# bxh1/VIDO-SLAM

Measured on AMD Instinct MI355X. Metric: frames/sec end-to-end (flow+depth+track+local-BA) at 640x480; BA iters/sec, higher is better.
Workload: dtype f32

## Files before the change

### include/vido_c.h

```cpp
#ifndef VIDO_C_H
#define VIDO_C_H
#include <stdint.h>
#include <stddef.h>
#ifdef __cplusplus
extern "C" {
#endif

#define VIDO_OK              0
#define VIDO_E_INVALID      -1
#define VIDO_E_NO_DEVICE    -2
#define VIDO_E_HIP          -3
#define VIDO_E_CAPACITY     -4
#define VIDO_E_NOMEM        -5

#define VIDO_MAX_LEVELS 16

typedef struct vido_ctx vido_ctx;

typedef struct vido_keypoint { float x, y, size, angle, response; int32_t octave; } vido_keypoint;

typedef struct vido_config {
    int32_t device;
    int32_t width, height;
    int32_t max_batch;
// ... 179 lines not shown
int vido_mask_logit_select_n(vido_ctx* ctx, const float* feat, const float* w, const float* b, const long long* labels, float* out, int n, int c, int hw, int classes, const int32_t* n_live);
int vido_bias_act(vido_ctx* ctx, float* x, const float* bias, int N, int C, int H, int W, float slope);
int vido_bias_unary(vido_ctx* ctx, float* x, const float* bias, int N, int C, int H, int W, int kind);
int vido_upcat_reflect(vido_ctx* ctx, const float* x, const float* skip, int C1, int C2, int h, int w, float* out);
int vido_minmax_norm_u16(vido_ctx* ctx, const float* d, const float* mm, int64_t n, int32_t* out);
int vido_bias_res_act(vido_ctx* ctx, float* x, const float* bias, const float* res, int N, int C, int H, int W, float slope);
int vido_area_feed(vido_ctx* ctx, const uint8_t* bgr, int H, int W, float* out, int OH, int OW, float div);
int vido_backwarp(vido_ctx* ctx, const float* x, const float* flow, int B, int C, int H, int W, float* out);
int vido_deconv4s2_depthwise(vido_ctx* ctx, const float* x, const float* weight, int B, int C, int H, int W, float input_slope, float* out);

int vido_conv1x1_supported(int cin, int cout, int hw);
int vido_conv1x1_layout(int cin, int cout, int hw);
int vido_conv1x1_set_arith(int arith);
int vido_conv1x1_range_flag(vido_ctx* ctx, int reset);
int vido_range_latch(vido_ctx* ctx, unsigned* dst);
int vido_conv1x1_bias_act(vido_ctx* ctx, const float* x, const float* w_packed, const float* bias, const float* residual, float* y, int cin, int cout, int hw, float slope);
int vido_deconv2x2_supported(int n, int cin, int cout, int h, int w);
int vido_deconv2x2_bias_act(vido_ctx* ctx, const float* x, const float* w_packed, const float* bias, float* y, int n, int cin, int cout, int h, int w, float slope);
int vido_deconv2x2_bias_act_n(vido_ctx* ctx, const float* x, const float* w_packed, const float* bias, float* y, int n, int cin, int cout, int h, int w, float slope, const int32_t* n_live);
int vido_conv1x1_bias_up2_act(vido_ctx* ctx, const float* x, const float* w_packed, const float* bias, const float* residual_half, float* y, int cin, int cout, int h, int w, float slope);

int vido_conv_kxk_c2(vido_ctx* ctx, const float* x, const float* w, const float* bias, const float* residual, float* y, int cin, int k, int h, int w_);
int vido_conv1x1_skinny(vido_ctx* ctx, const float* x, const float* w_packed, const float* bias, const float* residual, float* y, int cin, int cout, long long hw, float slope);
int vido_stem7x7s2_pool(vido_ctx* ctx, const float* x, const float* w_packed, const float* bias, float* y, int h, int w);

int vido_conv_direct_supported(int cin, int cout, int h, int w, int kh, int kw, int sh, int sw, int ph, int pw);
long long vido_conv_direct_packed_floats(int cin, int cout, int kh, int kw);
int vido_conv_direct_pack(const float* w, int cin, int cout, int kh, int kw, float* w_packed);
int vido_conv_direct_bias_act(vido_ctx* ctx, const float* x, const float* w_packed, const float* bias, float* y, int n, int cin, int cout, int h, int w,
                              int kh, int kw, int sh, int sw, int ph, int pw, float slope);

int vido_wino3x3_supported(int cin, int cout, int h, int w);
int vido_wino3x3_fills_chip(int n, int cout, int h, int w, int min_wgs);
long long vido_wino3x3_packed_floats(int cin, int cout);
int vido_wino3x3_pack(const float* w, int cin, int cout, float* u_packed);
int vido_wino3x3_bias_act(vido_ctx* ctx, const float* x, const float* u_packed, const float* bias, float* y, int n, int cin, int cout, int h, int w, float slope);
int vido_wino3x3_form(int n, int cin, int cout, int h, int w);
int vido_fc_h_splitk(int rows, int k, int outs);
int vido_fc_h(vido_ctx* ctx, const float* x, const void* w_packed, const float* bias, float* part, float* y, int rows, int k, int outs, float slope);
int vido_conv3x3_h_supported(int n, int cin, int cout, int h, int w);
int vido_conv3x3_h_workgroups(int n, int cout, int h, int w);
int vido_conv3x3_h_bias_act(vido_ctx* ctx, const float* x, const void* w_packed, const float* bias, float* y, int n, int cin, int cout, int h, int w, float slope);
int vido_conv3x3_h_bias_act_n(vido_ctx* ctx, const float* x, const void* w_packed, const float* bias, float* y, int n, int cin, int cout, int h, int w, float slope, const int32_t* n_live);
int vido_conv3x3_h_live_form(int n, int cout, int h, int w, int live, int* channels, int* block_rows);
int vido_mask_head_coarse(void);
int vido_conv3x3_h_bias_act_form(vido_ctx* ctx, const float* x, const void* w_packed, const float* bias, float* y, int n, int cin, int cout, int h, int w, float slope, int rpw, int cg);
long long vido_wino3x3_packed_floats_form(int cin, int cout, int form);
int vido_wino3x3_pack_form(const float* w, int cin, int cout, int form, float* u_packed);
int vido_wino3x3_bias_act_form(vido_ctx* ctx, const float* x, const float* u_packed, const float* bias, float* y, int n, int cin, int cout, int h, int w, float slope, int form);
int vido_gconv3x3_supported(int H, int W, int cpg_in, int cpg_out);
int64_t vido_gconv3x3_packed_size(int groups, int cpg_in, int cpg_out);
int vido_gconv3x3_bias_act(vido_ctx* ctx, const float* x, const float* in_bias, const float* w_packed, const float* bias, float* y, int groups, int cpg_in, int cpg_out, int H, int W, float slope);
int vido_gconv3x3_s2_supported(int H, int W, int cpg_in, int cpg_out);
int vido_gconv3x3_s2_bias_act(vido_ctx* ctx, const float* x, const float* w_packed, const float* bias, float* y, int groups, int cpg_in, int cpg_out, int H, int W, float slope);
int vido_lfn_reg_front(vido_ctx* ctx, const float* im1, const float* im2, const float* flow, const float* mean, float scale, int B, int C, int H, int W, float* out, int out_channels);
int vido_lfn_reg_tail(vido_ctx* ctx, const float* dist, const float* flow, const float* wx, const float* bx, const float* wy, const float* by, int B, int K, int H, int W, float* out);
int vido_roi_align(vido_ctx* ctx, const float* feat, int B, int C, int H, int W, const float* rois, int n_rois,
                   float spatial_scale, int pooled_h, int pooled_w, int sampling_ratio, float* out, int on_device);
int vido_nms(vido_ctx* ctx, const float* boxes_xyxy, const float* scores, int n, float thresh, int32_t* keep_out,
             int32_t* n_keep, int on_device);
int vido_nms_grouped(vido_ctx* ctx, const float* boxes_xyxy, const float* scores, const int32_t* groups, int n, float thresh,
                     int32_t* keep_out, int32_t* n_keep, int on_device);
int vido_nms_segments(vido_ctx* ctx, const float* boxes_xyxy, const int32_t* groups, const int32_t* seg_off, const int32_t* seg_n, int n_seg, int max_n, int total,
                      float thresh, int32_t* keep_out, int32_t* n_keep);
int vido_roi_align_fpn(vido_ctx* ctx, const float* const feat[4], const int H[4], const int W[4], const float scale[4], int C, const float* boxes, const int32_t* level,
                       int n, int pooled_h, int pooled_w, int sampling_ratio, float* out);
int vido_nchw_to_nhwc(vido_ctx* ctx, const float* src, int B, int C, int H, int W, float* dst);
int vido_roi_align_fpn_nhwc(vido_ctx* ctx, const float* const feat[4], const int H[4], const int W[4], const float scale[4], int C, const float* boxes, const int32_t* level,
                            int n, int pooled_h, int pooled_w, int sampling_ratio, float* out);
// ... 97 lines not shown
```

### vido-slam_amd/csrc/conv3x3h.hip

```cpp
#include "common.hpp"
#include <type_traits>

namespace {
typedef float f32x16 __attribute__((ext_vector_type(16)));
typedef float f32x2 __attribute__((ext_vector_type(2)));
typedef _Float16 f16x8 __attribute__((ext_vector_type(8)));
typedef _Float16 f16x2 __attribute__((ext_vector_type(2)));
typedef unsigned u32x4 __attribute__((ext_vector_type(4)));

#define C3_OOB 0x40000000u
#define C3_WSLOT 24576
#define C3_RBW 3
#define C3_WPIX(BR) (((BR) + 2) * 18)
#define C3_XP(BR) ((16 * C3_WPIX(BR) + 511) / 512)
#define C3_RAW(BR) (C3_XP(BR) * 8 * 256)
#define C3_PLANE(BR) (C3_WPIX(BR) * 32)
#define C3_PBUF(BR) (2 * C3_PLANE(BR))
#define C3_LDS(BR) (C3_RBW * C3_WSLOT + C3_RAW(BR) + 2 * C3_PBUF(BR))

struct C3Args { const float* x; const void* wp; const float* bias; float* y; int N, Cin, Cout, H, W, nby, nbx, mt, total, nchunk; float slope; unsigned wbytes; unsigned* range_flag; const int* n_live; };

template <int RPW, int CG>
__device__ __forceinline__ void c3_body(const C3Args& A, const int nby, const int nbx, const int mt, const int total, const int per)
{
    constexpr int BR = 16 / CG, MT = 32 * RPW * CG, WPIX = C3_WPIX(BR), XP = C3_XP(BR), RAWB = C3_RAW(BR), PLANE = C3_PLANE(BR), PBUF = C3_PBUF(BR), CK = (WPIX * 8 + 511) / 512, NMM = 9 * RPW, NRD = 2 * RPW + 2;
    extern __shared__ __attribute__((aligned(16))) char c3_lds[];
    char* L = c3_lds;
    const int tid = threadIdx.x, lane = tid & 63, w = __builtin_amdgcn_readfirstlane(tid >> 6);
    const int q8 = blockIdx.x >> 3, item = (blockIdx.x & 7) * per + q8;
    if (q8 >= per || item >= total) return;
    const int nt = item / mt, mtile = item - nt * mt, m0 = mtile * MT;
    const int bpi = nby * nbx, n = nt / bpi, brem = nt - n * bpi, by = brem / nbx, bx = brem - by * nbx, Y0 = by * BR, X0 = bx * 16;
    const int rp = CG == 1 ? w : (w & 3), rb0 = CG == 1 ? 0 : RPW * (w >> 2);
    const int hw = A.H * A.W, nsteps = A.nchunk * 3;

    const __amdgpu_buffer_rsrc_t wr = __builtin_amdgcn_make_buffer_rsrc((void*)A.wp, 0, A.wbytes, 0x00020000);
    const unsigned avo = 16u * (unsigned)lane;
    unsigned abase[3], avq[3];
#pragma unroll
    for (int q = 0; q < 3; q++) { const int i = w + 8 * q, rb = i / 6, rem = i - 6 * rb; abase[q] = 1024u * (unsigned)(((m0 >> 5) + rb) * A.nchunk * 18 + rem); avq[q] = rb < RPW * CG ? avo : 0x80000000u; }
    unsigned xvo[11];
#pragma unroll
    for (int j = 0; j < XP; j++) {
        const int e = 64 * (8 * j + w) + lane, ch = e / WPIX, rem = e - ch * WPIX, row = rem / 18, col = rem - row * 18, gy = Y0 - 1 + row, gx = X0 - 1 + col;
        xvo[j] = (e < 16 * WPIX && gy >= 0 && gy < A.H && gx >= 0 && gx < A.W) ? 4u * (unsigned)(ch * hw + gy * A.W + gx) : C3_OOB;
    }
    const unsigned ximg = 4u * (unsigned)n * (unsigned)A.Cin * (unsigned)hw, ximg_end = ximg + 4u * (unsigned)A.Cin * (unsigned)hw, xchunk = 64u * (unsigned)hw;
    char* const RAW = L + C3_RBW * C3_WSLOT;
    char* const PL = RAW + RAWB;
    auto issue_w = [&](int s, int slot) {
        char* S = L + slot * C3_WSLOT + w * 1024;
        const unsigned so = 6144u * (unsigned)s;
// ... 103 lines not shown
    const bool inside = Y < A.H && X < A.W;
    float* yb = A.y + (size_t)n * A.Cout * hw + (size_t)Y * A.W + X;
#pragma unroll
    for (int rb = 0; rb < RPW; rb++) {
        float bv[16], sv[16];
#pragma unroll
        for (int r = 0; r < 16; r++) { const int co = m0 + 32 * (rb0 + rb) + 8 * (r >> 2) + 4 * (lane >> 5) + (r & 3); bv[r] = A.bias ? A.bias[co] : 0.f; sv[r] = wsc[co]; }
        if (inside) {
#pragma unroll
            for (int r = 0; r < 16; r++) {
                const int co = m0 + 32 * (rb0 + rb) + 8 * (r >> 2) + 4 * (lane >> 5) + (r & 3);
                const float v = acc[rb][r] * sv[r] + bv[r];
                yb[(size_t)co * hw] = fmaxf(v, v * A.slope);
            }
        }
    }
}

template <int RPW, int CG>
__global__ __launch_bounds__(512) void k_conv3x3_h(C3Args A)
{
    int total = A.total, per = gridDim.x >> 3;
    if (A.n_live) { const int nl = min(max(*A.n_live, 0), A.N); total = nl * A.nby * A.nbx * A.mt; per = (total + 7) >> 3; }
    c3_body<RPW, CG>(A, A.nby, A.nbx, A.mt, total, per);
}

#define C3_FINE_RPW 1
#define C3_FINE_CG 2
template <int RPWC, int CGC>
__global__ __launch_bounds__(512) void k_conv3x3_h_live(C3Args A, int fine_max)
{
    constexpr int BRF = 16 / C3_FINE_CG, MTF = 32 * C3_FINE_RPW * C3_FINE_CG, BRC = 16 / CGC, MTC = 32 * RPWC * CGC;
    const int nl = min(max(*A.n_live, 0), A.N), nbx = (A.W + 15) >> 4;
    const int nbyf = (A.H + BRF - 1) / BRF, mtf = A.Cout / MTF, tf = nl * nbyf * nbx * mtf;
    if (tf <= fine_max) c3_body<C3_FINE_RPW, C3_FINE_CG>(A, nbyf, nbx, mtf, tf, (tf + 7) >> 3);
    else { const int nbyc = (A.H + BRC - 1) / BRC, mtc = A.Cout / MTC, tc = nl * nbyc * nbx * mtc; c3_body<RPWC, CGC>(A, nbyc, nbx, mtc, tc, (tc + 7) >> 3); }
}
}

extern "C" {

int vido_conv3x3_h_supported(int n, int cin, int cout, int h, int w)
{
    const long long cp = (cin + 15) / 16 * 16;
    return n >= 1 && cin >= 1 && (cout == 32 || cout == 64 || (cout >= 128 && cout % 128 == 0)) && h >= 1 && w >= 1 && 4ll * n * cin * h * w < (1ll << 30) && 4ll * n * cout * h * w < (1ll << 30)
           && 36ll * cp * cout < (1ll << 31);
}

#define C3_MIN16 190
static int c3_block_rows(int n, int cout, int h, int w)
{
    static const int force = [] { const char* e = getenv("VIDO_CONV3X3_H_ROWS"); return e ? atoi(e) : 0; }();
    if (cout == 32) return 16;
    if (force == 16 || force == 8) return force;
    const int mt = cout >= 128 ? cout / 128 : 1;
    return n * ((h + 15) / 16) * ((w + 15) / 16) * mt >= C3_MIN16 ? 16 : 8;
}
int vido_conv3x3_h_workgroups(int n, int cout, int h, int w) { const int br = c3_block_rows(n, cout, h, w); return n * ((h + br - 1) / br) * ((w + 15) / 16) * (cout >= 128 ? cout / 128 : 1); }

// ... 67 lines not shown
    return VIDO_OK;
}

int vido_conv3x3_h_bias_act_form(vido_ctx* ctx, const float* x, const void* w_packed, const float* bias, float* y, int n, int cin, int cout, int h, int w, float slope, int rpw, int cg)
{
    if (!ctx) return VIDO_E_INVALID;
    const int MT = 32 * rpw * cg, form = rpw * 10 + cg;
    if (!x || !w_packed || !y || x == y || !vido_conv3x3_h_supported(n, cin, cout, h, w) || slope < 0.f || slope > 1.f || (((uintptr_t)x | (uintptr_t)y) & 3) || ((uintptr_t)w_packed & 15)
        || (form != 41 && form != 22 && form != 21 && form != 12 && form != 11) || cout % MT)
        return vido_set_error(ctx, VIDO_E_INVALID, "conv3x3_h_form: no kernel <%d, %d> for %d x %d -> %d channels at %d x %d", rpw, cg, n, cin, cout, h, w);
    HIP_TRY(ctx, hipSetDevice(ctx->device));
    { int rc = c3_set_attrs(ctx); if (rc) return rc; }
    hipStream_t st = ctx->has_ext_stream ? ctx->ext_stream : ctx->stream;
    const int br = 16 / cg, nby = (h + br - 1) / br, nbx = (w + 15) / 16, mt = cout / MT, total = n * nby * nbx * mt, nchunk = (cin + 15) / 16;
    C3Args A{x, w_packed, bias, y, n, cin, cout, h, w, nby, nbx, mt, total, nchunk, slope, (unsigned)(36ll * 16 * nchunk * cout), ctx->c1_range_flag, nullptr};
    const dim3 grid(8 * ((total + 7) / 8));
#define C3_LAUNCH(RPW_, CG_) hipLaunchKernelGGL((k_conv3x3_h<RPW_, CG_>), grid, dim3(512), C3_LDS(16 / CG_), st, A)
    if (form == 41) C3_LAUNCH(4, 1); else if (form == 22) C3_LAUNCH(2, 2); else if (form == 21) C3_LAUNCH(2, 1); else if (form == 12) C3_LAUNCH(1, 2); else C3_LAUNCH(1, 1);
#undef C3_LAUNCH
    HIP_TRY(ctx, hipGetLastError());
    return VIDO_OK;
}

}
```

### vido-slam_amd/csrc/convsmall.hip

```cpp
#include "common.hpp"

namespace {
template <int K>
__global__ __launch_bounds__(256) void k_conv_kxk_c2(const float* __restrict__ x, const float* __restrict__ w, const float* __restrict__ bias, const float* __restrict__ res,
                                                     float* __restrict__ y, int Cin, int H, int W)
{
    constexpr int R = K / 2, TS = 16 + K - 1, CC = 8, NT = CC * TS * TS, NL = (NT + 255) / 256, NW = (CC * K * K * 2 + 255) / 256;
    __shared__ float tile[NT];
    __shared__ __attribute__((aligned(8))) float wl[NW * 256];
    const int tid = threadIdx.x, tx = tid & 15, ty = tid >> 4, bx = blockIdx.x * 16, by = blockIdx.y * 16;
    const size_t HW = (size_t)H * W;
    int toff[NL]; bool tin[NL]; int tch[NL];
#pragma unroll
    for (int j = 0; j < NL; j++) {
        const int i = min(tid + 256 * j, NT - 1), c = i / (TS * TS), r = i - c * (TS * TS), yy = r / TS, xx = r - yy * TS, gy = by + yy - R, gx = bx + xx - R;
        tch[j] = c; tin[j] = tid + 256 * j < NT && gy >= 0 && gy < H && gx >= 0 && gx < W;
        toff[j] = min(max(gy, 0), H - 1) * W + min(max(gx, 0), W - 1);
    }
    float tv[NL], wv[NW];
    auto fetch = [&](int c0) {
#pragma unroll
        for (int j = 0; j < NL; j++) { const int c = min(c0 + tch[j], Cin - 1); tv[j] = x[(size_t)c * HW + toff[j]]; }
#pragma unroll
        for (int j = 0; j < NW; j++) {
// ... 14 lines not shown
#pragma unroll 2
        for (int c = 0; c < CC; c++) {
            const float* tc = tile + c * TS * TS + ty * TS + tx;
            const float2* wc = (const float2*)wl + c * K * K;
#pragma unroll
            for (int dy = 0; dy < K; dy++)
#pragma unroll
                for (int dx = 0; dx < K; dx++) {
                    const float v = tc[dy * TS + dx];
                    const float2 ww = wc[dy * K + dx];
                    acc0 = fmaf(v, ww.x, acc0); acc1 = fmaf(v, ww.y, acc1);
                }
        }
    }
    const int gy = by + ty, gx = bx + tx;
    if (gy < H && gx < W) {
        const size_t o = (size_t)gy * W + gx;
        y[o] = acc0 + (res ? res[o] : 0.f); y[HW + o] = acc1 + (res ? res[HW + o] : 0.f);
    }
}

typedef float f32x16s __attribute__((ext_vector_type(16)));
template <int CB, bool RES, int D>
__global__ __launch_bounds__(256) void k_conv1x1_skinny(const float* __restrict__ x, const float* __restrict__ wp, const float* __restrict__ bias, const float* __restrict__ res,
                                                        float* __restrict__ y, int Cin, int Cout, long long HW, float slope, unsigned xbytes, unsigned wbytes)
{
    const int lane = threadIdx.x & 63, wv = __builtin_amdgcn_readfirstlane(threadIdx.x >> 6);
    const long long p0 = ((long long)blockIdx.x * 4 + wv) * 32;
    if (p0 >= HW) return;
    const long long p = min(p0 + (lane & 31), HW - 1);
    const int nkp = Cin >> 1;
    f32x16s acc[CB];
#pragma unroll
    for (int cb = 0; cb < CB; cb++)
#pragma unroll
        for (int r = 0; r < 16; r++) acc[cb][r] = 0.f;
    const __amdgpu_buffer_rsrc_t xr = __builtin_amdgcn_make_buffer_rsrc((void*)x, 0, xbytes, 0x00020000);
    const __amdgpu_buffer_rsrc_t wr = __builtin_amdgcn_make_buffer_rsrc((void*)wp, 0, wbytes, 0x00020000);
    const unsigned xvo = 4u * (unsigned)((lane >> 5) * HW + p), wvo = 4u * (unsigned)lane;
    const unsigned hw8 = 8u * (unsigned)HW;
    float b[D], a[D][CB], bn[D], an[D][CB];
    auto fetch = [&](int kp0, float (&fb)[D], float (&fa)[D][CB]) {
#pragma unroll
        for (int u = 0; u < D; u++) {
            const int kp = min(kp0 + u, nkp - 1);
            fb[u] = __builtin_bit_cast(float, __builtin_amdgcn_raw_buffer_load_b32(xr, xvo, hw8 * (unsigned)kp, 0));
#pragma unroll
            for (int cb = 0; cb < CB; cb++) fa[u][cb] = __builtin_bit_cast(float, __builtin_amdgcn_raw_buffer_load_b32(wr, wvo, 256u * (unsigned)(cb * nkp + kp), 0));
        }
    };
    constexpr bool AHEAD = D > 4;
// ... 13 lines not shown
                b[u] = bn[u];
#pragma unroll
                for (int cb = 0; cb < CB; cb++) a[u][cb] = an[u][cb];
            }
        }
    }
    if (p0 + (lane & 31) < HW) {
#pragma unroll
        for (int cb = 0; cb < CB; cb++) {
            float bv[16], rv[16];
#pragma unroll
            for (int r = 0; r < 16; r++) {
                const int co = min(cb * 32 + 8 * (r >> 2) + 4 * (lane >> 5) + (r & 3), Cout - 1);
                bv[r] = bias ? bias[co] : 0.f; rv[r] = RES ? res[(size_t)co * HW + p] : 0.f;
            }
#pragma unroll
            for (int r = 0; r < 16; r++) {
                const int co = cb * 32 + 8 * (r >> 2) + 4 * (lane >> 5) + (r & 3);
                const float v = acc[cb][r] + bv[r] + rv[r];
                if (co < Cout) y[(size_t)co * HW + p] = fmaxf(v, v * slope);
            }
        }
    }
}
}

extern "C" {

int vido_conv_kxk_c2(vido_ctx* ctx, const float* x, const float* w, const float* bias, const float* residual, float* y, int cin, int k, int h, int wd)
{
    if (!ctx) return VIDO_E_INVALID;
    if (!x || !w || !y || x == y || cin < 1 || h < 1 || wd < 1 || (k != 3 && k != 5 && k != 7)) return vido_set_error(ctx, VIDO_E_INVALID, "conv_kxk_c2: bad arguments (k = %d)", k);
    HIP_TRY(ctx, hipSetDevice(ctx->device));
    hipStream_t st = ctx->has_ext_stream ? ctx->ext_stream : ctx->stream;
    const dim3 grid((wd + 15) / 16, (h + 15) / 16), blk(256);
    if (k == 7) hipLaunchKernelGGL(k_conv_kxk_c2<7>, grid, blk, 0, st, x, w, bias, residual, y, cin, h, wd);
    else if (k == 5) hipLaunchKernelGGL(k_conv_kxk_c2<5>, grid, blk, 0, st, x, w, bias, residual, y, cin, h, wd);
    else hipLaunchKernelGGL(k_conv_kxk_c2<3>, grid, blk, 0, st, x, w, bias, residual, y, cin, h, wd);
    HIP_TRY(ctx, hipGetLastError());
    return VIDO_OK;
}

int vido_conv1x1_skinny(vido_ctx* ctx, const float* x, const float* w_packed, const float* bias, const float* residual, float* y, int cin, int cout, long long hw, float slope)
{
    if (!ctx) return VIDO_E_INVALID;
    if (!x || !w_packed || !y || x == y || cin < 2 || (cin & 1) || cin > 256 || cout < 1 || cout > 256 || hw < 1 || slope < 0.f || slope > 1.f || 4ll * cin * hw >= (1ll << 32))
        return vido_set_error(ctx, VIDO_E_INVALID, "conv1x1_skinny: no kernel for %d -> %d channels", cin, cout);
    HIP_TRY(ctx, hipSetDevice(ctx->device));
    hipStream_t st = ctx->has_ext_stream ? ctx->ext_stream : ctx->stream;
    const dim3 grid((unsigned)((hw + 127) / 128)), blk(256);
    const int cbn = (cout + 31) / 32;
    const unsigned xb = (unsigned)(4ll * cin * hw), wb = (unsigned)(4ll * cbn * 32 * cin);
    int depth = 16;
    if (const char* e = getenv("VIDO_SKINNY_DEPTH")) {
        depth = atoi(e);
        if (depth != 4 && depth != 8 && depth != 16) return vido_set_error(ctx, VIDO_E_INVALID, "conv1x1_skinny: VIDO_SKINNY_DEPTH=%s (4, 8 or 16)", e);
    }
#define SK_LAUNCH(CBV, DV) { if (residual) hipLaunchKernelGGL((k_conv1x1_skinny<CBV, true, DV>), grid, blk, 0, st, x, w_packed, bias, residual, y, cin, cout, hw, slope, xb, wb); \
                             else hipLaunchKernelGGL((k_conv1x1_skinny<CBV, false, DV>), grid, blk, 0, st, x, w_packed, bias, residual, y, cin, cout, hw, slope, xb, wb); }
    switch (cbn) {
    case 1: if (depth == 4) SK_LAUNCH(1, 4) else if (depth == 8) SK_LAUNCH(1, 8) else SK_LAUNCH(1, 16) break;
    case 2: SK_LAUNCH(2, 4) break; case 3: SK_LAUNCH(3, 4) break; case 4: SK_LAUNCH(4, 4) break;
    case 5: SK_LAUNCH(5, 4) break; case 6: SK_LAUNCH(6, 4) break; case 7: SK_LAUNCH(7, 4) break; default: SK_LAUNCH(8, 4) break;
    }
#undef SK_LAUNCH
    HIP_TRY(ctx, hipGetLastError());
    return VIDO_OK;
}

}
```

### vido-slam_amd/nets/maskrcnn.py

```python
import math
import os
from collections import OrderedDict
from dataclasses import dataclass
import numpy as np
import torch
import torch.nn as nn
import torch.nn.functional as F


@dataclass
class MaskRCNNConfig:
    blocks: tuple = (3, 4, 23, 3)
    groups: int = 32
    width_per_group: int = 8
    stride_in_1x1: bool = False
    stem_out: int = 64
    res2_out: int = 256
    fpn_out: int = 256
    anchor_sizes: tuple = (32, 64, 128, 256, 512)
    aspect_ratios: tuple = (0.5, 1.0, 2.0)
    anchor_strides: tuple = (4, 8, 16, 32, 64)
    pre_nms_top_n: int = 1000
    post_nms_top_n: int = 1000
    fpn_post_nms_top_n: int = 1000
# ... 131 lines not shown
    def _layer(self, i, x):
        conv = getattr(self, "fpn_layer%d" % i)
        if self._ops is not None and x.is_cuda and hasattr(self._ops, "wino3x3_conv") and not os.environ.get("VIDO_NO_WINO"):
            y = self._ops.wino3x3_conv(conv, x, 1.0)
            if y is not None:
                return y
        return conv(x)

    def _inner(self, i, x, top=None):
        conv = getattr(self, "fpn_inner%d" % i)
        if self._ops is not None and x.is_cuda and hasattr(self._ops, "conv1x1_conv") and not os.environ.get("VIDO_NO_CONV1X1"):
            if top is None:
                y = self._ops.conv1x1_conv(conv, x, 1.0)
            elif x.shape[2] % 2 == 0 and x.shape[3] % 2 == 0 and tuple(top.shape[2:]) == (x.shape[2] // 2, x.shape[3] // 2):
                y = self._ops.conv1x1_conv(conv, x, 1.0, residual_up2=top)
            else:
                y = None
            if y is not None:
                return y
        y = conv(x)
        return y if top is None else y + F.interpolate(top, scale_factor=2, mode="nearest")

    def forward(self, feats):
        inner = self._inner(self.n, feats[-1])
        out = [self._layer(self.n, inner)]
        for i in range(self.n - 1, 0, -1):
            inner = self._inner(i, feats[i - 1], inner)
            out.insert(0, self._layer(i, inner))
        out.append(F.max_pool2d(out[-1], 1, 2, 0))
        return out


def cell_anchors(stride, size, ratios):
    base = np.array([0.0, 0.0, stride - 1.0, stride - 1.0])
    w, h = base[2] - base[0] + 1, base[3] - base[1] + 1
    xc, yc = base[0] + 0.5 * (w - 1), base[1] + 0.5 * (h - 1)
    ws = np.round(np.sqrt(w * h / np.asarray(ratios, np.float64))); hs = np.round(ws * np.asarray(ratios, np.float64))
    s = float(size) / stride
    rows = [[xc - 0.5 * (a * s - 1), yc - 0.5 * (b * s - 1), xc + 0.5 * (a * s - 1), yc + 0.5 * (b * s - 1)] for a, b in zip(ws, hs)]
    return torch.from_numpy(np.asarray(rows, np.float64)).float()


class _Buffers(nn.Module):
    def __init__(self, tensors):
        super().__init__()
        for i, t in enumerate(tensors):
            self.register_buffer(str(i), t)

    def __iter__(self):
        return iter(self._buffers.values())

# ... 3 lines not shown
        super().__init__()
        self.strides = c.anchor_strides
        self.cell_anchors = _Buffers([cell_anchors(st, sz, c.aspect_ratios) for st, sz in zip(c.anchor_strides, c.anchor_sizes)])

    def forward(self, grid_sizes):
        out = []
        for (gh, gw), stride, base in zip(grid_sizes, self.strides, self.cell_anchors):
            sx = torch.arange(0, gw * stride, step=stride, dtype=torch.float32, device=base.device)
            sy = torch.arange(0, gh * stride, step=stride, dtype=torch.float32, device=base.device)
            yy, xx = torch.meshgrid(sy, sx, indexing="ij")
            shifts = torch.stack((xx.reshape(-1), yy.reshape(-1), xx.reshape(-1), yy.reshape(-1)), 1)
            out.append((shifts.view(-1, 1, 4) + base.view(1, -1, 4)).reshape(-1, 4))
        return out


class _RPNHead(nn.Module):
    def __init__(self, ch, na):
        super().__init__()
        self.conv = nn.Conv2d(ch, ch, 3, 1, 1); self.cls_logits = nn.Conv2d(ch, na, 1); self.bbox_pred = nn.Conv2d(ch, na * 4, 1)

    _ops = None

    def forward(self, feats):
        t = [_conv_bias_relu(self.conv, f, self._ops) for f in feats]
        ops = self._ops
        if ops is not None and t[0].is_cuda and hasattr(ops, "conv1x1_skinny") and not os.environ.get("VIDO_NO_CONVSMALL") and t[0].shape[0] == 1 and self.conv.out_channels % 2 == 0 and self.conv.out_channels <= 256:
            from .ops import pack_conv1x1_skinny
            key = (self.cls_logits.weight.data_ptr(), self.cls_logits.weight._version, self.bbox_pred.weight.data_ptr(), self.bbox_pred.weight._version, str(t[0].device))
            if getattr(self, "_head_key", None) != key:
                self._head_w = pack_conv1x1_skinny(torch.cat([self.cls_logits.weight, self.bbox_pred.weight], 0)).to(t[0].device)
                self._head_b = torch.cat([self.cls_logits.bias, self.bbox_pred.bias], 0).detach().contiguous(); self._head_key = key
            na = self.cls_logits.out_channels; nt = na + self.bbox_pred.out_channels
            ys = [ops.conv1x1_skinny(x, self._head_w, self._head_b, nt, 1.0) for x in t]
            return [y[:, :na] for y in ys], [y[:, na:] for y in ys]
        return [self.cls_logits(x) for x in t], [self.bbox_pred(x) for x in t]


def _conv_bias_relu(conv, x, ops, n_live=None):
    if ops is None or not x.is_cuda or conv.bias is None:
        return F.relu(conv(x))
    if isinstance(conv, nn.Conv2d) and hasattr(ops, "wino3x3_conv") and not os.environ.get("VIDO_NO_WINO"):
        y = ops.wino3x3_conv(conv, x, 0.0, n_live=n_live) if n_live is not None else ops.wino3x3_conv(conv, x, 0.0)
        if y is not None:
            return y
    if isinstance(conv, nn.ConvTranspose2d) and hasattr(ops, "deconv2x2_conv"):
        y = ops.deconv2x2_conv(conv, x, 0.0, n_live) if n_live is not None else ops.deconv2x2_conv(conv, x, 0.0)
        if y is not None:
            return y
    if isinstance(conv, nn.ConvTranspose2d):
        y = F.conv_transpose2d(x, conv.weight, None, conv.stride, conv.padding, conv.output_padding, conv.groups, conv.dilation)
    else:
        y = F.conv2d(x, conv.weight, None, conv.stride, conv.padding, conv.dilation, conv.groups)
    return ops.bias_act_(y.contiguous(), conv.bias, 0.0)


def clip_boxes(b, w, h):
# ... 502 lines not shown
```

### vido-slam_amd/nets/ops.py

```python
import contextlib
import ctypes as C
import os
import torch

_WINO_MIN_WGS = int(os.environ.get("VIDO_WINO_MIN_WGS", "0"))
_CONV3X3_H_MIN_WGS = 0 if os.environ.get("VIDO_CONV3X3_H") == "0" else int(os.environ.get("VIDO_CONV3X3_H_MIN_WGS", "128"))
_CONVDIRECT_SET = os.environ.get("VIDO_CONVDIRECT_SET", "novalu")


def correlation_torch_reference(first, second, stride):
    a, b = first[:, :, ::stride, ::stride], second[:, :, ::stride, ::stride]
    pad = torch.nn.functional.pad(b, (3, 3, 3, 3))
    H, W = a.shape[2], a.shape[3]
    return torch.stack([(a * pad[:, :, p:p + H, o:o + W]).mean(1) for p in range(7) for o in range(7)], 1)


class HipOps:

    _range_safe = 0

    def __init__(self, ctx):
        self.ctx = ctx

    @property
    def range_safe_active(self):
        return self._range_safe > 0

    @staticmethod
    def _live_ptr(n_live):
        if n_live is None:
# ... 310 lines not shown
        form = self.wino3x3_form(x.shape[0], w.shape[1], w.shape[0], x.shape[2], x.shape[3])
        key = (w.data_ptr(), w._version, str(x.device))
        if getattr(conv, "_wino_key", None) != key:
            conv._wino_u = {}; conv._wino_key = key
        if form not in conv._wino_u:
            conv._wino_u[form] = pack_wino3x3(w, form).to(x.device)
        return self.wino3x3_bias_act(x.contiguous(), conv._wino_u[form], b, int(w.shape[0]), slope, form)

    def conv3x3_h_bias_act(self, x, w_packed, bias, cout, slope, n_live=None):
        assert x.is_cuda and x.is_contiguous() and x.dtype == torch.float32
        N, cin, H, W = x.shape
        assert w_packed.dtype == torch.int16 and w_packed.numel() == 2 * cout * ((cin + 15) // 16 * 16 * 9 + 1), "conv3x3_h: weight not packed by pack_conv3x3_h for this layer"
        out = torch.empty((N, cout, H, W), device=x.device, dtype=torch.float32)
        self.gconv_flops = getattr(self, "gconv_flops", 0.0) + 2.0 * N * cout * cin * 9 * H * W
        self._adopt_stream()
        self.ctx._check(self.ctx.lib.vido_conv3x3_h_bias_act_n(self.ctx.h, C.c_void_p(x.data_ptr()), C.c_void_p(w_packed.data_ptr()), C.c_void_p(bias.data_ptr()) if bias is not None else None,
                                                               C.c_void_p(out.data_ptr()), int(N), int(cin), int(cout), int(H), int(W), C.c_float(slope), self._live_ptr(n_live)))
        return out

    def conv3x3_h_live_form(self, n, cout, h, w, live):
        ch, br = C.c_int(), C.c_int()
        fine = self.ctx.lib.vido_conv3x3_h_live_form(int(n), int(cout), int(h), int(w), int(live), C.byref(ch), C.byref(br))
        return bool(fine), ch.value, br.value

    def fc_h(self, x, w_packed, bias, outs, slope=1.0):
        assert x.is_cuda and x.is_contiguous() and x.dtype == torch.float32 and x.dim() == 2
        rows, k = int(x.shape[0]), int(x.shape[1])
        S = int(self.ctx.lib.vido_fc_h_splitk(rows, k, int(outs)))
        if S <= 0:
            return None
        assert w_packed.dtype == torch.int16 and w_packed.numel() == 2 * outs * (k + 1), "fc_h: weight not packed (pack_conv1x1(w[:, :, None, None], 3))"
        part = torch.empty((S, rows, outs), device=x.device, dtype=torch.float32); y = torch.empty((rows, outs), device=x.device, dtype=torch.float32)
        self.gconv_flops = getattr(self, "gconv_flops", 0.0) + 2.0 * rows * k * outs
        self._adopt_stream()
        self.ctx._check(self.ctx.lib.vido_fc_h(self.ctx.h, C.c_void_p(x.data_ptr()), C.c_void_p(w_packed.data_ptr()), C.c_void_p(bias.data_ptr()) if bias is not None else None,
                                               C.c_void_p(part.data_ptr()), C.c_void_p(y.data_ptr()), rows, k, int(outs), C.c_float(slope)))
        return y

    def fc_h_linear(self, lin, x, slope=1.0):
        w = lin.weight
        if not x.is_cuda or x.dtype != torch.float32 or x.dim() != 2 or os.environ.get("VIDO_NO_FC_H") or self._range_safe or int(self.ctx.lib.vido_fc_h_splitk(int(x.shape[0]), int(w.shape[1]), int(w.shape[0]))) <= 0:
            return None
        key = (w.data_ptr(), w._version, str(x.device))
        if getattr(lin, "_fch_key", None) != key:
            lin._fch_w = pack_conv1x1(w.detach().reshape(int(w.shape[0]), int(w.shape[1]), 1, 1), 3).to(x.device); lin._fch_key = key
        return self.fc_h(x.contiguous(), lin._fch_w, lin.bias, int(w.shape[0]), slope)
# ... 643 lines not shown
```

Measured before the change: 130.4.

## Batch FPN/RPN pyramid levels into grouped multi-problem conv launches

Adds multi-problem kernels that launch the 3x3 conv for several pyramid levels (FPN output layers, RPN shared conv) in one grid, plus a grouped 1x1 skinny head kernel over all RPN levels. A fit routine packs smaller levels into the idle compute-unit tail left by the largest level, so small levels stop running as separate under-occupied launches. The goals are fewer kernel launches and better occupancy on small maps. The cost is a per-block dispatch over a kernel-argument struct, extra host-side planning and ctypes overhead, and FPN inner computation being reordered ahead of the layer convs.

```diff
diff --git a/include/vido_c.h b/include/vido_c.h
--- a/include/vido_c.h
+++ b/include/vido_c.h
@@ -225,6 +225,7 @@
 
 int vido_conv_kxk_c2(vido_ctx* ctx, const float* x, const float* w, const float* bias, const float* residual, float* y, int cin, int k, int h, int w_);
 int vido_conv1x1_skinny(vido_ctx* ctx, const float* x, const float* w_packed, const float* bias, const float* residual, float* y, int cin, int cout, long long hw, float slope);
+int vido_conv1x1_skinny_multi(vido_ctx* ctx, int np, const float* const* x, const float* w_packed, const float* bias, float* const* y, const long long* hw, int cin, int cout, float slope);
 int vido_stem7x7s2_pool(vido_ctx* ctx, const float* x, const float* w_packed, const float* bias, float* y, int h, int w);
 
 int vido_conv_direct_supported(int cin, int cout, int h, int w, int kh, int kw, int sh, int sw, int ph, int pw);
@@ -248,6 +249,10 @@
 int vido_conv3x3_h_live_form(int n, int cout, int h, int w, int live, int* channels, int* block_rows);
 int vido_mask_head_coarse(void);
 int vido_conv3x3_h_bias_act_form(vido_ctx* ctx, const float* x, const void* w_packed, const float* bias, float* y, int n, int cin, int cout, int h, int w, float slope, int rpw, int cg);
+int vido_conv3x3_h_bias_act_multi(vido_ctx* ctx, int np, const float* const* x, const void* const* w_packed, const float* const* bias, float* const* y, const int* h, const int* w,
+                                  int cin, int cout, float slope);
+int vido_conv3x3_h_multi_plan(int np, const int* h, const int* w, int cout, int* first_out);
+int vido_conv3x3_h_multi_fit(int np, const int* h, const int* w, int cout, int cus, int min_wgs, int* take_out);
 long long vido_wino3x3_packed_floats_form(int cin, int cout, int form);
 int vido_wino3x3_pack_form(const float* w, int cin, int cout, int form, float* u_packed);
 int vido_wino3x3_bias_act_form(vido_ctx* ctx, const float* x, const float* u_packed, const float* bias, float* y, int n, int cin, int cout, int h, int w, float slope, int form);
diff --git a/vido-slam_amd/csrc/conv3x3h.hip b/vido-slam_amd/csrc/conv3x3h.hip
--- a/vido-slam_amd/csrc/conv3x3h.hip
+++ b/vido-slam_amd/csrc/conv3x3h.hip
@@ -21,13 +21,13 @@
 struct C3Args { const float* x; const void* wp; const float* bias; float* y; int N, Cin, Cout, H, W, nby, nbx, mt, total, nchunk; float slope; unsigned wbytes; unsigned* range_flag; const int* n_live; };
 
 template <int RPW, int CG>
-__device__ __forceinline__ void c3_body(const C3Args& A, const int nby, const int nbx, const int mt, const int total, const int per)
+__device__ __forceinline__ void c3_body(const C3Args& A, const int bid, const int nby, const int nbx, const int mt, const int total, const int per)
 {
     constexpr int BR = 16 / CG, MT = 32 * RPW * CG, WPIX = C3_WPIX(BR), XP = C3_XP(BR), RAWB = C3_RAW(BR), PLANE = C3_PLANE(BR), PBUF = C3_PBUF(BR), CK = (WPIX * 8 + 511) / 512, NMM = 9 * RPW, NRD = 2 * RPW + 2;
     extern __shared__ __attribute__((aligned(16))) char c3_lds[];
     char* L = c3_lds;
     const int tid = threadIdx.x, lane = tid & 63, w = __builtin_amdgcn_readfirstlane(tid >> 6);
-    const int q8 = blockIdx.x >> 3, item = (blockIdx.x & 7) * per + q8;
+    const int q8 = bid >> 3, item = (bid & 7) * per + q8;
     if (q8 >= per || item >= total) return;
     const int nt = item / mt, mtile = item - nt * mt, m0 = mtile * MT;
     const int bpi = nby * nbx, n = nt / bpi, brem = nt - n * bpi, by = brem / nbx, bx = brem - by * nbx, Y0 = by * BR, X0 = bx * 16;
@@ -177,7 +177,7 @@
 {
     int total = A.total, per = gridDim.x >> 3;
     if (A.n_live) { const int nl = min(max(*A.n_live, 0), A.N); total = nl * A.nby * A.nbx * A.mt; per = (total + 7) >> 3; }
-    c3_body<RPW, CG>(A, A.nby, A.nbx, A.mt, total, per);
+    c3_body<RPW, CG>(A, (int)blockIdx.x, A.nby, A.nbx, A.mt, total, per);
 }
 
 #define C3_FINE_RPW 1
@@ -188,8 +188,22 @@
     constexpr int BRF = 16 / C3_FINE_CG, MTF = 32 * C3_FINE_RPW * C3_FINE_CG, BRC = 16 / CGC, MTC = 32 * RPWC * CGC;
     const int nl = min(max(*A.n_live, 0), A.N), nbx = (A.W + 15) >> 4;
     const int nbyf = (A.H + BRF - 1) / BRF, mtf = A.Cout / MTF, tf = nl * nbyf * nbx * mtf;
-    if (tf <= fine_max) c3_body<C3_FINE_RPW, C3_FINE_CG>(A, nbyf, nbx, mtf, tf, (tf + 7) >> 3);
-    else { const int nbyc = (A.H + BRC - 1) / BRC, mtc = A.Cout / MTC, tc = nl * nbyc * nbx * mtc; c3_body<RPWC, CGC>(A, nbyc, nbx, mtc, tc, (tc + 7) >> 3); }
+    if (tf <= fine_max) c3_body<C3_FINE_RPW, C3_FINE_CG>(A, (int)blockIdx.x, nbyf, nbx, mtf, tf, (tf + 7) >> 3);
+    else { const int nbyc = (A.H + BRC - 1) / BRC, mtc = A.Cout / MTC, tc = nl * nbyc * nbx * mtc; c3_body<RPWC, CGC>(A, (int)blockIdx.x, nbyc, nbx, mtc, tc, (tc + 7) >> 3); }
+}
+
+#define C3_MULTI_MAX 6
+struct C3Multi { C3Args a[C3_MULTI_MAX]; int first[C3_MULTI_MAX + 1]; int np; };
+template <int RPW, int CG>
+__global__ __launch_bounds__(512) void k_conv3x3_h_multi(C3Multi M)
+{
+    const int b = (int)blockIdx.x;
+    C3Args A = M.a[0];
+    int f = 0, e = M.first[1];
+#pragma unroll
+    for (int k = 1; k < C3_MULTI_MAX; k++)
+        if (k < M.np && b >= M.first[k]) { A = M.a[k]; f = M.first[k]; e = M.first[k + 1]; }
+    c3_body<RPW, CG>(A, b - f, A.nby, A.nbx, A.mt, A.total, (e - f) >> 3);
 }
 }
 
@@ -303,4 +317,83 @@
     return VIDO_OK;
 }
 
-}
+static long long c3_multi_wgs(int cout, int h, int w) { return (long long)((h + 15) / 16) * ((w + 15) / 16) * (cout / 128); }
+static bool c3_multi_shape_ok(int np, const int* h, const int* w, int cout)
+{
+    if (np < 1 || np > C3_MULTI_MAX || !h || !w || cout < 128 || cout % 128) return false;
+    long long sum = 0;
+    for (int j = 0; j < np; j++) {
+        if (h[j] < 1 || w[j] < 1 || 4ll * cout * h[j] * w[j] >= (1ll << 30)) return false;
+        sum += 8 * ((c3_multi_wgs(cout, h[j], w[j]) + 7) / 8);
+    }
+    return sum < (1ll << 30);
+}
+
+int vido_conv3x3_h_multi_plan(int np, const int* h, const int* w, int cout, int* first_out)
+{
+    if (!c3_multi_shape_ok(np, h, w, cout)) return -1;
+    int f = 0;
+    for (int j = 0; j < np; j++) {
+        if (first_out) first_out[j] = f;
+        f += (int)(8 * ((c3_multi_wgs(cout, h[j], w[j]) + 7) / 8));
+    }
+    if (first_out) first_out[np] = f;
+    return f;
+}
+
+int vido_conv3x3_h_multi_fit(int np, const int* h, const int* w, int cout, int cus, int min_wgs, int* take_out)
+{
+    if (take_out) for (int j = 0; j < np && j < 64; j++) take_out[j] = 0;
+    if (np < 1 || np > 64 || !h || !w || cus < 1 || cout < 128 || cout % 128) return 0;
+    for (int j = 0; j < np; j++) if (h[j] < 1 || w[j] < 1 || 4ll * cout * h[j] * w[j] >= (1ll << 30)) return 0;
+    const long long w0 = c3_multi_wgs(cout, h[0], w[0]);
+    if (w0 < std::max(min_wgs, 1)) return 0;
+    const long long room = (w0 + cus - 1) / cus * cus;
+    long long used = w0;
+    int taken = 1;
+    if (take_out) take_out[0] = 1;
+    for (int j = 1; j < np && taken < C3_MULTI_MAX; j++) {
+        const long long wj = c3_multi_wgs(cout, h[j], w[j]);
+        if (used + wj <= room) { used += wj; taken++; if (take_out) take_out[j] = 1; }
+    }
+    return taken;
+}
+
+int vido_conv3x3_h_bias_act_multi(vido_ctx* ctx, int np, const float* const* x, const void* const* w_packed, const float* const* bias, float* const* y, const int* h, const int* w,
+                                  int cin, int cout, float slope)
+{
+    if (!ctx) return VIDO_E_INVALID;
+    if (!x || !w_packed || !y || !c3_multi_shape_ok(np, h, w, cout) || slope < 0.f || slope > 1.f)
+        return vido_set_error(ctx, VIDO_E_INVALID, "conv3x3_h_multi: %d problems (1..%d), cout %d (a multiple of 128), or a map without kernel, or slope outside [0, 1]", np, C3_MULTI_MAX, cout);
+    for (int j = 0; j < np; j++) {
+        if (!x[j] || !w_packed[j] || !y[j] || x[j] == y[j] || !vido_conv3x3_h_supported(1, cin, cout, h[j], w[j]) || (((uintptr_t)x[j] | (uintptr_t)y[j]) & 3) || ((uintptr_t)w_packed[j] & 15))
+            return vido_set_error(ctx, VIDO_E_INVALID, "conv3x3_h_multi: problem %d: no kernel for %d -> %d channels at %d x %d (or a pointer is null, misaligned, or x == y)", j, cin, cout, h[j], w[j]);
+        const uintptr_t y0 = (uintptr_t)y[j], y1 = y0 + 4ull * cout * h[j] * w[j];
+        for (int k = 0; k < np; k++) {
+            const uintptr_t x0 = (uintptr_t)x[k], x1 = x0 + 4ull * cin * h[k] * w[k], z0 = (uintptr_t)y[k], z1 = z0 + 4ull * cout * h[k] * w[k];
+            if ((y0 < x1 && x0 < y1) || (k != j && y0 < z1 && z0 < y1))
+                return vido_set_error(ctx, VIDO_E_INVALID, "conv3x3_h_multi: the output of problem %d overlaps the %s of problem %d", j, (y0 < x1 && x0 < y1) ? "input" : "output", k);
+        }
+    }
+    HIP_TRY(ctx, hipSetDevice(ctx->device));
+    hipStream_t st = ctx->has_ext_stream ? ctx->ext_stream : ctx->stream;
+    static bool attr[64] = {};
+    if (!attr[ctx->device & 63]) {
+        HIP_TRY(ctx, hipFuncSetAttribute((const void*)k_conv3x3_h_multi<4, 1>, hipFuncAttributeMaxDynamicSharedMemorySize, (int)C3_LDS(16)));
+        attr[ctx->device & 63] = true;
+    }
+    C3Multi M{};
+    const int nchunk = (cin + 15) / 16, mt = cout / 128;
+    M.np = np;
+    const int grid = vido_conv3x3_h_multi_plan(np, h, w, cout, M.first);
+    for (int j = np + 1; j <= C3_MULTI_MAX; j++) M.first[j] = grid;
+    for (int j = 0; j < np; j++) {
+        const int nby = (h[j] + 15) / 16, nbx = (w[j] + 15) / 16;
+        M.a[j] = C3Args{x[j], w_packed[j], bias ? bias[j] : nullptr, y[j], 1, cin, cout, h[j], w[j], nby, nbx, mt, nby * nbx * mt, nchunk, slope, (unsigned)(36ll * 16 * nchunk * cout), ctx->c1_range_flag, nullptr};
+    }
+    hipLaunchKernelGGL((k_conv3x3_h_multi<4, 1>), dim3((unsigned)grid), dim3(512), C3_LDS(16), st, M);
+    HIP_TRY(ctx, hipGetLastError());
+    return VIDO_OK;
+}
+
+}
diff --git a/vido-slam_amd/csrc/convsmall.hip b/vido-slam_amd/csrc/convsmall.hip
--- a/vido-slam_amd/csrc/convsmall.hip
+++ b/vido-slam_amd/csrc/convsmall.hip
@@ -60,11 +60,11 @@
 
 typedef float f32x16s __attribute__((ext_vector_type(16)));
 template <int CB, bool RES, int D>
-__global__ __launch_bounds__(256) void k_conv1x1_skinny(const float* __restrict__ x, const float* __restrict__ wp, const float* __restrict__ bias, const float* __restrict__ res,
-                                                        float* __restrict__ y, int Cin, int Cout, long long HW, float slope, unsigned xbytes, unsigned wbytes)
+__device__ __forceinline__ void sk_body(const float* __restrict__ x, const float* __restrict__ wp, const float* __restrict__ bias, const float* __restrict__ res,
+                                        float* __restrict__ y, const int Cin, const int Cout, const long long HW, const float slope, const unsigned xbytes, const unsigned wbytes, const int bid)
 {
     const int lane = threadIdx.x & 63, wv = __builtin_amdgcn_readfirstlane(threadIdx.x >> 6);
-    const long long p0 = ((long long)blockIdx.x * 4 + wv) * 32;
+    const long long p0 = ((long long)bid * 4 + wv) * 32;
     if (p0 >= HW) return;
     const long long p = min(p0 + (lane & 31), HW - 1);
     const int nkp = Cin >> 1;
@@ -124,6 +124,26 @@
             }
         }
     }
+}
+
+template <int CB, bool RES, int D>
+__global__ __launch_bounds__(256) void k_conv1x1_skinny(const float* __restrict__ x, const float* __restrict__ wp, const float* __restrict__ bias, const float* __restrict__ res,
+                                                        float* __restrict__ y, int Cin, int Cout, long long HW, float slope, unsigned xbytes, unsigned wbytes)
+{
+    sk_body<CB, RES, D>(x, wp, bias, res, y, Cin, Cout, HW, slope, xbytes, wbytes, (int)blockIdx.x);
+}
+
+#define SK_MULTI_MAX 8
+struct SkMulti { const float* x[SK_MULTI_MAX]; float* y[SK_MULTI_MAX]; long long hw[SK_MULTI_MAX]; unsigned xbytes[SK_MULTI_MAX]; int first[SK_MULTI_MAX + 1]; int np; };
+template <int D>
+__global__ __launch_bounds__(256) void k_conv1x1_skinny_multi(SkMulti M, const float* __restrict__ wp, const float* __restrict__ bias, int Cin, int Cout, float slope, unsigned wbytes)
+{
+    const int b = (int)blockIdx.x;
+    const float* x = M.x[0]; float* y = M.y[0]; long long hw = M.hw[0]; unsigned xb = M.xbytes[0]; int f = 0;
+#pragma unroll
+    for (int k = 1; k < SK_MULTI_MAX; k++)
+        if (k < M.np && b >= M.first[k]) { x = M.x[k]; y = M.y[k]; hw = M.hw[k]; xb = M.xbytes[k]; f = M.first[k]; }
+    sk_body<1, false, D>(x, wp, bias, nullptr, y, Cin, Cout, hw, slope, xb, wbytes, b - f);
 }
 }
 
@@ -170,4 +190,43 @@
     return VIDO_OK;
 }
 
-}
+int vido_conv1x1_skinny_multi(vido_ctx* ctx, int np, const float* const* x, const float* w_packed, const float* bias, float* const* y, const long long* hw, int cin, int cout, float slope)
+{
+    if (!ctx) return VIDO_E_INVALID;
+    if (np < 1 || np > SK_MULTI_MAX || !x || !w_packed || !y || !hw || cin < 2 || (cin & 1) || cin > 256 || cout < 1 || cout > 32 || slope < 0.f || slope > 1.f)
+        return vido_set_error(ctx, VIDO_E_INVALID, "conv1x1_skinny_multi: %d maps (1..%d), no kernel for %d -> %d channels (cout <= 32)", np, SK_MULTI_MAX, cin, cout);
+    SkMulti M{};
+    long long blocks = 0;
+    for (int j = 0; j < np; j++) {
+        if (!x[j] || !y[j] || x[j] == y[j] || hw[j] < 1 || 4ll * cin * hw[j] >= (1ll << 32))
+            return vido_set_error(ctx, VIDO_E_INVALID, "conv1x1_skinny_multi: map %d: null pointer, x == y or %lld positions", j, hw[j]);
+        const uintptr_t y0 = (uintptr_t)y[j], y1 = y0 + 4ull * cout * hw[j];
+        for (int k = 0; k < np; k++) {
+            if (hw[k] < 1) continue;
+            const uintptr_t x0 = (uintptr_t)x[k], x1 = x0 + 4ull * cin * hw[k], z0 = (uintptr_t)y[k], z1 = z0 + 4ull * cout * hw[k];
+            if ((y0 < x1 && x0 < y1) || (k != j && y0 < z1 && z0 < y1))
+                return vido_set_error(ctx, VIDO_E_INVALID, "conv1x1_skinny_multi: the output of map %d overlaps the %s of map %d", j, (y0 < x1 && x0 < y1) ? "input" : "output", k);
+        }
+        M.x[j] = x[j]; M.y[j] = y[j]; M.hw[j] = hw[j]; M.xbytes[j] = (unsigned)(4ll * cin * hw[j]); M.first[j] = (int)blocks;
+        blocks += (hw[j] + 127) / 128;
+        if (blocks >= (1ll << 30)) return vido_set_error(ctx, VIDO_E_INVALID, "conv1x1_skinny_multi: too many positions");
+    }
+    for (int j = np; j <= SK_MULTI_MAX; j++) M.first[j] = (int)blocks;
+    M.np = np;
+    int depth = 16;
+    if (const char* e = getenv("VIDO_SKINNY_DEPTH")) {
+        depth = atoi(e);
+        if (depth != 4 && depth != 8 && depth != 16) return vido_set_error(ctx, VIDO_E_INVALID, "conv1x1_skinny_multi: VIDO_SKINNY_DEPTH=%s (4, 8 or 16)", e);
+    }
+    HIP_TRY(ctx, hipSetDevice(ctx->device));
+    hipStream_t st = ctx->has_ext_stream ? ctx->ext_stream : ctx->stream;
+    const dim3 grid((unsigned)blocks), blk(256);
+    const unsigned wb = (unsigned)(4ll * 32 * cin);
+    if (depth == 4) hipLaunchKernelGGL((k_conv1x1_skinny_multi<4>), grid, blk, 0, st, M, w_packed, bias, cin, cout, slope, wb);
+    else if (depth == 8) hipLaunchKernelGGL((k_conv1x1_skinny_multi<8>), grid, blk, 0, st, M, w_packed, bias, cin, cout, slope, wb);
+    else hipLaunchKernelGGL((k_conv1x1_skinny_multi<16>), grid, blk, 0, st, M, w_packed, bias, cin, cout, slope, wb);
+    HIP_TRY(ctx, hipGetLastError());
+    return VIDO_OK;
+}
+
+}
diff --git a/vido-slam_amd/nets/maskrcnn.py b/vido-slam_amd/nets/maskrcnn.py
--- a/vido-slam_amd/nets/maskrcnn.py
+++ b/vido-slam_amd/nets/maskrcnn.py
@@ -177,11 +177,16 @@
         return y if top is None else y + F.interpolate(top, scale_factor=2, mode="nearest")
 
     def forward(self, feats):
-        inner = self._inner(self.n, feats[-1])
-        out = [self._layer(self.n, inner)]
+        inner = [None] * self.n
+        inner[self.n - 1] = self._inner(self.n, feats[-1])
         for i in range(self.n - 1, 0, -1):
-            inner = self._inner(i, feats[i - 1], inner)
-            out.insert(0, self._layer(i, inner))
+            inner[i - 1] = self._inner(i, feats[i - 1], inner[i])
+        ops = self._ops; done = {}
+        if ops is not None and self.n >= 3 and inner[0].is_cuda and hasattr(ops, "conv3x3_h_group") and not os.environ.get("VIDO_NO_WINO"):
+            cand = [0] + list(range(2, self.n))
+            got = ops.conv3x3_h_group([getattr(self, "fpn_layer%d" % (i + 1)) for i in cand], [inner[i] for i in cand], 1.0, "fpn")
+            done = {cand[k]: y for k, y in got.items()}
+        out = [done[i] if i in done else self._layer(i + 1, inner[i]) for i in range(self.n)]
         out.append(F.max_pool2d(out[-1], 1, 2, 0))
         return out
 
@@ -231,8 +236,12 @@
     _ops = None
 
     def forward(self, feats):
-        t = [_conv_bias_relu(self.conv, f, self._ops) for f in feats]
-        ops = self._ops
+        ops = self._ops; done = {}
+        if ops is not None and len(feats) >= 3 and feats[0].is_cuda and hasattr(ops, "conv3x3_h_group") and self.conv.bias is not None and not os.environ.get("VIDO_NO_WINO"):
+            cand = [0] + list(range(2, len(feats)))
+            got = ops.conv3x3_h_group(self.conv, [feats[i] for i in cand], 0.0, "rpn")
+            done = {cand[k]: y for k, y in got.items()}
+        t = [done[i] if i in done else _conv_bias_relu(self.conv, f, self._ops) for i, f in enumerate(feats)]
         if ops is not None and t[0].is_cuda and hasattr(ops, "conv1x1_skinny") and not os.environ.get("VIDO_NO_CONVSMALL") and t[0].shape[0] == 1 and self.conv.out_channels % 2 == 0 and self.conv.out_channels <= 256:
             from .ops import pack_conv1x1_skinny
             key = (self.cls_logits.weight.data_ptr(), self.cls_logits.weight._version, self.bbox_pred.weight.data_ptr(), self.bbox_pred.weight._version, str(t[0].device))
@@ -240,7 +249,11 @@
                 self._head_w = pack_conv1x1_skinny(torch.cat([self.cls_logits.weight, self.bbox_pred.weight], 0)).to(t[0].device)
                 self._head_b = torch.cat([self.cls_logits.bias, self.bbox_pred.bias], 0).detach().contiguous(); self._head_key = key
             na = self.cls_logits.out_channels; nt = na + self.bbox_pred.out_channels
-            ys = [ops.conv1x1_skinny(x, self._head_w, self._head_b, nt, 1.0) for x in t]
+            from .ops import level_groups_off
+            if hasattr(ops, "conv1x1_skinny_multi") and 2 <= len(t) <= 8 and nt <= 32 and not level_groups_off("heads") and not getattr(ops, "_range_safe", 0):
+                ys = ops.conv1x1_skinny_multi(t, self._head_w, self._head_b, nt, 1.0)
+            else:
+                ys = [ops.conv1x1_skinny(x, self._head_w, self._head_b, nt, 1.0) for x in t]
             return [y[:, :na] for y in ys], [y[:, na:] for y in ys]
         return [self.cls_logits(x) for x in t], [self.bbox_pred(x) for x in t]
 
diff --git a/vido-slam_amd/nets/ops.py b/vido-slam_amd/nets/ops.py
--- a/vido-slam_amd/nets/ops.py
+++ b/vido-slam_amd/nets/ops.py
@@ -6,6 +6,33 @@
 _WINO_MIN_WGS = int(os.environ.get("VIDO_WINO_MIN_WGS", "0"))
 _CONV3X3_H_MIN_WGS = 0 if os.environ.get("VIDO_CONV3X3_H") == "0" else int(os.environ.get("VIDO_CONV3X3_H_MIN_WGS", "128"))
 _CONVDIRECT_SET = os.environ.get("VIDO_CONVDIRECT_SET", "novalu")
+
+
+def level_groups_off(part):
+    v = os.environ.get("VIDO_NO_LEVEL_GROUPS")
+    if not v or v == "0":
+        return False
+    names = [s.strip() for s in v.split(",")]
+    return part in names if set(names) <= {"fpn", "rpn", "heads"} else True
+
+
+def _lib_of(lib):
+    if lib is None:
+        from ..host import load_library
+        lib = load_library()
+    return lib
+
+
+def conv3x3_h_multi_plan(sizes, cout, lib=None):
+    lib = _lib_of(lib); n = len(sizes); I = C.c_int * max(n, 1); first = (C.c_int * (n + 1))()
+    g = int(lib.vido_conv3x3_h_multi_plan(n, I(*[int(s[0]) for s in sizes]), I(*[int(s[1]) for s in sizes]), int(cout), first))
+    return (g, list(first)) if g >= 0 else (-1, None)
+
+
+def conv3x3_h_multi_fit(sizes, cout, cus, min_wgs=None, lib=None):
+    lib = _lib_of(lib); n = len(sizes); I = C.c_int * max(n, 1); take = I()
+    got = int(lib.vido_conv3x3_h_multi_fit(n, I(*[int(s[0]) for s in sizes]), I(*[int(s[1]) for s in sizes]), int(cout), int(cus), int(_CONV3X3_H_MIN_WGS if min_wgs is None else min_wgs), take))
+    return got, list(take)[:n]
 
 
 def correlation_torch_reference(first, second, stride):
@@ -362,6 +389,74 @@
         ch, br = C.c_int(), C.c_int()
         fine = self.ctx.lib.vido_conv3x3_h_live_form(int(n), int(cout), int(h), int(w), int(live), C.byref(ch), C.byref(br))
         return bool(fine), ch.value, br.value
+
+    def conv3x3_h_multi(self, xs, w_packed, bias, cout, slope):
+        n = len(xs)
+        wps = list(w_packed) if isinstance(w_packed, (list, tuple)) else [w_packed] * n
+        bs = list(bias) if isinstance(bias, (list, tuple)) else [bias] * n
+        assert len(wps) == n and len(bs) == n
+        xs = [x.contiguous() for x in xs]
+        cin = int(xs[0].shape[1]) if n else 0
+        for x, wp in zip(xs, wps):
+            assert x.is_cuda and x.dtype == torch.float32 and x.dim() == 4 and x.shape[0] == 1 and int(x.shape[1]) == cin
+            assert wp.dtype == torch.int16 and wp.numel() == 2 * cout * ((cin + 15) // 16 * 16 * 9 + 1), "conv3x3_h: weight not packed by pack_conv3x3_h for this layer"
+        outs = [torch.empty((1, cout, x.shape[2], x.shape[3]), device=x.device, dtype=torch.float32) for x in xs]
+        self.gconv_flops = getattr(self, "gconv_flops", 0.0) + sum(2.0 * cout * cin * 9 * x.shape[2] * x.shape[3] for x in xs)
+        P = C.c_void_p * max(n, 1); I = C.c_int * max(n, 1)
+        self._adopt_stream()
+        self.ctx._check(self.ctx.lib.vido_conv3x3_h_bias_act_multi(
+            self.ctx.h, n, P(*[x.data_ptr() for x in xs]), P(*[w.data_ptr() for w in wps]), P(*[b.data_ptr() if b is not None else None for b in bs]),
+            P(*[y.data_ptr() for y in outs]), I(*[int(x.shape[2]) for x in xs]), I(*[int(x.shape[3]) for x in xs]), int(cin), int(cout), C.c_float(slope)))
+        return outs
+
+    def conv3x3_h_multi_plan(self, sizes, cout):
+        return conv3x3_h_multi_plan(sizes, cout, self.ctx.lib)
+
+    def level_group(self, convs, xs, part):
+        if level_groups_off(part) or self._range_safe or _CONV3X3_H_MIN_WGS <= 0 or len(xs) < 2:
+            return None
+        convs = list(convs) if isinstance(convs, (list, tuple)) else [convs] * len(xs)
+        w0 = convs[0].weight
+        cout, cin = int(w0.shape[0]), int(w0.shape[1])
+        for conv, x in zip(convs, xs):
+            w = conv.weight
+            if (tuple(w.shape) != (cout, cin, 3, 3) or tuple(conv.stride) != (1, 1) or tuple(conv.padding) != (1, 1) or tuple(conv.dilation) != (1, 1) or conv.groups != 1
+                    or getattr(conv, "padding_mode", "zeros") != "zeros" or not x.is_cuda or x.dtype != torch.float32 or x.dim() != 4 or x.shape[0] != 1 or int(x.shape[1]) != cin
+                    or not self.ctx.lib.vido_conv3x3_h_supported(1, cin, cout, int(x.shape[2]), int(x.shape[3]))):
+                return None
+        order = sorted(range(len(xs)), key=lambda i: -int(xs[i].shape[2]) * int(xs[i].shape[3]))
+        n = len(order); I = C.c_int * n; take = I()
+        cus = int(torch.cuda.get_device_properties(xs[0].device).multi_processor_count)
+        got = self.ctx.lib.vido_conv3x3_h_multi_fit(n, I(*[int(xs[i].shape[2]) for i in order]), I(*[int(xs[i].shape[3]) for i in order]), cout, cus, int(_CONV3X3_H_MIN_WGS), take)
+        return [i for i, t in zip(order, take) if t] if got >= 2 else None
+
+    def conv3x3_h_group(self, convs, xs, slope, part):
+        idx = self.level_group(convs, xs, part)
+        if not idx:
+            return {}
+        convs = list(convs) if isinstance(convs, (list, tuple)) else [convs] * len(xs)
+        wps = []
+        for i in idx:
+            conv = convs[i]; w = conv.weight
+            key = (w.data_ptr(), w._version, str(xs[i].device))
+            if getattr(conv, "_c3h_key", None) != key:
+                conv._c3h_w = pack_conv3x3_h(w).to(xs[i].device); conv._c3h_key = key
+            wps.append(conv._c3h_w)
+        ys = self.conv3x3_h_multi([xs[i] for i in idx], wps, [convs[i].bias for i in idx], int(convs[0].weight.shape[0]), slope)
+        return dict(zip(idx, ys))
+
+    def conv1x1_skinny_multi(self, xs, w_packed, bias, cout, slope=1.0):
+        xs = [x.contiguous() for x in xs]
+        n = len(xs); cin = int(xs[0].shape[1]) if n else 0
+        for x in xs:
+            assert x.is_cuda and x.dtype == torch.float32 and x.dim() == 4 and x.shape[0] == 1 and int(x.shape[1]) == cin
+        outs = [torch.empty((1, cout, x.shape[2], x.shape[3]), device=x.device, dtype=torch.float32) for x in xs]
+        self.gconv_flops = getattr(self, "gconv_flops", 0.0) + sum(2.0 * cout * cin * x.shape[2] * x.shape[3] for x in xs)
+        P = C.c_void_p * max(n, 1); L = C.c_longlong * max(n, 1)
+        self._adopt_stream()
+        self.ctx._check(self.ctx.lib.vido_conv1x1_skinny_multi(self.ctx.h, n, P(*[x.data_ptr() for x in xs]), C.c_void_p(w_packed.data_ptr()), C.c_void_p(bias.data_ptr()) if bias is not None else None,
+                                                               P(*[y.data_ptr() for y in outs]), L(*[int(x.shape[2]) * int(x.shape[3]) for x in xs]), int(cin), int(cout), C.c_float(slope)))
+        return outs
 
     def fc_h(self, x, w_packed, bias, outs, slope=1.0):
         assert x.is_cuda and x.is_contiguous() and x.dtype == torch.float32 and x.dim() == 2
```

Result: no change. 129.7 (-0.5%).
